# ttaoREtw/semi-tts

Measured on AMD Instinct MI355X. Metric: mel-frames/sec (decode+attn), higher is better.
Workload: dtype f32

## Files before the change

semi_tts_amd/csrc/attention.hip:

```cpp
#include "attention_body.h"

namespace {

inline unsigned at_align_bits(const AtArgs& a, const void* ws) {
    return (st_aligned16(a.pm) ? ST_ATTN_AL_PM : 0) | (st_aligned16(a.pq) ? ST_ATTN_AL_PQ : 0) | (st_aligned16(a.v) ? ST_ATTN_AL_V : 0) |
           (st_aligned16(a.loc_lin_w) ? ST_ATTN_AL_WL : 0) | (st_aligned16(a.memory) ? ST_ATTN_AL_MEM : 0) |
           (st_aligned16(a.s_buf) ? ST_ATTN_AL_S : 0) | (st_aligned16(ws) ? ST_ATTN_AL_WS : 0);
}

template <int PART>
int at_launch(const AtArgs& a, hipStream_t stream) {
    const AtPlan pl = at_plan(PART, a.B, a.L, a.A, a.E, a.F, a.K, PART == 1 ? a.pre_parts : PART == 2 ? a.fin_parts : 1, at_align_bits(a, nullptr));
    ST_CHECK_ARG(pl.code != ST_ATTN_R_DIMS, "attention step: bad dims");
    ST_CHECK_ARG(pl.code != ST_ATTN_R_K_EVEN, "attention step: location kernel size %d must be odd", a.K);
    ST_CHECK_ARG(pl.code != ST_ATTN_R_PARTS, "attention step: parts=%d must be 1, 2, 4 or 8 with E=%d a multiple of 4*parts", a.fin_parts, a.E);
    ST_CHECK_ARG(pl.code != ST_ATTN_R_E, "attention step: E=%d must be a multiple of 4 and <= %d", a.E, 4 * AT_THREADS);
    ST_CHECK_ARG(pl.code != ST_ATTN_R_ALIGN, "attention step: memory, pm/pq/v and the S buffer must be 16-byte aligned");
    ST_CHECK_ARG(PART == 1 || a.ctx || a.ctx_dst[0].base, "attention step: no context output");
    ST_CHECK_ARG(PART == 0 || a.s_buf, "attention step: S buffer missing");
    ST_CHECK_ARG(!a.h_q || (a.ada_std && a.ada_mean && a.h_adapt), "attention step: AdaIN pointers");
    const size_t lds_bytes = pl.lds;
    ST_CHECK_ARG(pl.code != ST_ATTN_R_LDS, "attention step: L=%d needs %zu B of LDS (> 160 KiB)%s", a.L, lds_bytes,
                 PART == 0 ? "; the split form (st_attn_pre_fwd with more parts + st_attn_fin_fwd) takes longer texts" : "");
    ST_CHECK_ARG(pl.code == 0, "attention step: refused (%d)", pl.code);
    static size_t configured[2] = {0, 0};
    int rc = st_lds_opt_in(reinterpret_cast<const void*>(at_kernel<true, PART>), 160 * 1024, pl.opt_in, configured[0]);
    if (!rc) rc = st_lds_opt_in(reinterpret_cast<const void*>(at_kernel<false, PART>), 160 * 1024, pl.opt_in, configured[1]);
    if (rc) return rc;
    const bool vec = pl.vec;
    const int nwg = pl.nwg;
    if (vec) hipLaunchKernelGGL((at_kernel<true, PART>), dim3(nwg), dim3(AT_THREADS), lds_bytes, stream, a.pq, a.pm, a.v, a.w_cum_prev, a.memory,
                                a.s_buf, a.L, a.A, a.E, a.fin_parts, a);
    else hipLaunchKernelGGL((at_kernel<false, PART>), dim3(nwg), dim3(AT_THREADS), lds_bytes, stream, a.pq, a.pm, a.v, a.w_cum_prev, a.memory,
                            a.s_buf, a.L, a.A, a.E, a.fin_parts, a);
    ST_LAUNCH_CHECK();
    return 0;
}

struct AsArgs {
    const float* pq; const float* s_buf; const float* memory; const float* v;
    float* w_tmp; int ld_w;
    float* ws;
    int B, L, A, E, P, Lp;
};

__global__ __launch_bounds__(AT_THREADS) void at_split_kernel(const AsArgs a) {
    __shared__ float es[512];
    __shared__ __attribute__((aligned(16))) float part[4 * AT_THREADS];
    __shared__ float stat[2];
    const int tid = threadIdx.x, lane = tid & 63, wave = tid >> 6;
    const int b = blockIdx.x / a.P, p = blockIdx.x - b * a.P;
    const int L = a.L, A = a.A, E = a.E;
    const int l0 = p * a.Lp, l1 = min(L, l0 + a.Lp), n = l1 - l0;
    const float* sb = a.s_buf + ((size_t)b * L + l0) * A;
    const float* memb = a.memory + ((size_t)b * L + l0) * E;
    const int ne4 = E >> 2;
    const int ng = AT_THREADS / ne4, e4 = tid % ne4, g = tid / ne4;
    constexpr int PFR = 11;
    f32x4 mpf[PFR];
#pragma unroll
    for (int j = 0; j < PFR; ++j) {
        const int l = g + j * ng;
        mpf[j] = (g < ng && l < n) ? st_ld4(memb + (size_t)l * E + e4 * 4) : f32x4{0.f, 0.f, 0.f, 0.f};
    }
// ... 218 lines not shown
```

semi_tts_amd/csrc/attention_body.h:

```cpp
#pragma once
#include "st_common.h"

#ifndef AT_PROF
#define AT_PROF(n)
#endif

namespace {

constexpr int AT_THREADS = 512;
constexpr int AT_WAVES = AT_THREADS / 64;
constexpr int AT_PF = 12;
constexpr int AT_LB = 8;
constexpr int AT_LP = 6;
constexpr int AT_CB = 4;
constexpr int AT_WLPF = 4;

struct AtArgs {
    const float* pq; const float* pm; const float* memory;
    const float* w_prev; int ld_wprev; const float* w_cum_prev;
    float* w_out; int ld_wout; float* w_cum_out;
    const float* loc_conv_w; const float* loc_lin_w; const float* v;
    float* ctx; int ld_ctx; st_t16_view ctx_dst[3];
    const float* h_q; int ld_hq; const float* ada_std; const float* ada_mean; float* h_adapt; int Q;
    float* s_buf;
// ... 6 lines not shown
};

constexpr int AT_GRAN_SPINS = 1 << 18;
__device__ __forceinline__ f32x4 at_wait_granules(const unsigned long long* base, unsigned epoch, int lane, int A, unsigned* status,
                                                  int max_spins) {
    typedef __attribute__((address_space(1))) unsigned long long gu64;
    gu64* gp = (gu64*)(base + min(lane * 4, A - 4));
    unsigned long long g0 = 0, g1 = 0, g2 = 0, g3 = 0;
    bool ok = false;
    for (int spins = 0; spins < max_spins; ++spins) {
        g0 = __hip_atomic_load(gp + 0, __ATOMIC_RELAXED, __HIP_MEMORY_SCOPE_AGENT);
        g1 = __hip_atomic_load(gp + 1, __ATOMIC_RELAXED, __HIP_MEMORY_SCOPE_AGENT);
        g2 = __hip_atomic_load(gp + 2, __ATOMIC_RELAXED, __HIP_MEMORY_SCOPE_AGENT);
        g3 = __hip_atomic_load(gp + 3, __ATOMIC_RELAXED, __HIP_MEMORY_SCOPE_AGENT);
        const bool mine = (unsigned)(g0 >> 32) == epoch && (unsigned)(g1 >> 32) == epoch &&
                          (unsigned)(g2 >> 32) == epoch && (unsigned)(g3 >> 32) == epoch;
        ok = __all(mine);
        if (ok) break;
        __builtin_amdgcn_s_sleep(2);
    }
    if (!ok && lane == 0 && status) __hip_atomic_fetch_or(status, 1u, __ATOMIC_RELAXED, __HIP_MEMORY_SCOPE_AGENT);
    const float nanv = __builtin_nanf("");
    return ok ? f32x4{__uint_as_float((unsigned)g0), __uint_as_float((unsigned)g1), __uint_as_float((unsigned)g2),
                      __uint_as_float((unsigned)g3)}
              : f32x4{nanv, nanv, nanv, nanv};
}

struct AtLds {
    int wt, wt_ld, wc, kp, hs, hl, cf, cf_ld, e, part, total;
};

__host__ __device__ inline int at_pos_per(int L, int nparts) {
    return nparts > 1 ? (((L + nparts - 1) / nparts + 11) / 12) * 12 : L;
}

__host__ __device__ inline AtLds at_layout(int L, int A, int E, int F, int K, int part = 0, int Lr = 0, bool pre_mfma = false) {
    AtLds o;
    int p = 0;
    const int Lh = part == 1 ? Lr : L;
    o.wt_ld = ((A + 3) & ~3) + 4;
    o.wt = p; if (part == 0 || (part == 1 && !pre_mfma)) p += F * o.wt_ld;
    o.kp = K <= 32 ? 32 : ((K + 3) & ~3);
    o.wc = p; if (part != 2) p += F * 2 * o.kp;
    o.hl = ((Lh + AT_CB + o.kp + 3) + 3) & ~3;
    o.hs = p; if (part != 2) p += 2 * o.hl;
    o.cf_ld = ((((Lh + AT_LP - 1) / AT_LP) * AT_LP + AT_CB + 3) & ~3) + (part == 1 ? 16 : 0);
    o.cf = p; if (part != 2) p += F * o.cf_ld;
    o.e = p; p += ((L + 3) & ~3);
    o.part = p; p += 4 * AT_THREADS;
    o.total = p;
    return o;
}

__device__ __forceinline__ float at_tanh(float x) {
    const float t = __expf(-2.0f * fabsf(x));
    return copysignf(__fdividef(1.0f - t, 1.0f + t), x);
}

__device__ __forceinline__ size_t at_t16_off(int b, int k, int KB) {
    return (((size_t)(b >> 4) * KB + (k >> 4)) * 64 + ((k >> 2) & 3) * 16 + (b & 15)) * 4 + (k & 3);
}

__device__ __forceinline__ void at_put_granule(unsigned long long* p, float v, unsigned epoch) {
    typedef __attribute__((address_space(1))) unsigned long long gu64;
    __hip_atomic_store((gu64*)p, ((unsigned long long)epoch << 32) | (unsigned long long)__float_as_uint(v), __ATOMIC_RELAXED,
                       __HIP_MEMORY_SCOPE_AGENT);
// ... 111 lines not shown
        float s = 0.0f;
        for (int gg = 0; gg < ng; ++gg) s += part[gg * E + e];
        at_put_granule(xme + e, s, a.epoch);
    }
    const int Es = E / P;
    if (wave < P) {
        const unsigned long long* xq = a.xchg + ((size_t)b * P + wave) * (E + 4);
        const f32x4 st4 = at_wait_granules(xq + E, a.epoch, lane, 4, a.status, AT_GRAN_SPINS);
        const f32x4 c4 = at_wait_granules(xq + (size_t)p * Es, a.epoch, lane, Es, a.status, AT_GRAN_SPINS);
        if (lane * 4 < Es) *reinterpret_cast<f32x4*>(cb + wave * 256 + lane * 4) = c4;
        if (lane == 0) { gst[2 * wave] = st4[0]; gst[2 * wave + 1] = st4[1]; }
    }
    __syncthreads();
    float M = -INFINITY;
    for (int q = 0; q < P; ++q) M = fmaxf(M, gst[2 * q]);
    float D = 0.0f;
    for (int q = 0; q < P; ++q) D += gst[2 * q + 1] * __expf(gst[2 * q] - M);
    if (tid < Es) {
        float s = 0.0f;
        for (int q = 0; q < P; ++q) s = fmaf(__expf(gst[2 * q] - M) / D, cb[q * 256 + tid], s);
        const int e = p * Es + tid;
#pragma unroll
        for (int d = 0; d < 3; ++d)
            if (a.ctx_dst[d].base) a.ctx_dst[d].base[at_t16_off(b, a.ctx_dst[d].kb0 * 16 + e, a.ctx_dst[d].kb_stride)] = s;
    }
    const float scp = __expf(stat[0] - M) / D;
    for (int l = tid; l < n; l += NT) {
        const float w = es[l] * scp;
        a.w_out[(size_t)b * a.ld_wout + l0 + l] = w;
        a.w_cum_out[(size_t)b * L + l0 + l] = w + a.w_cum_prev[(size_t)b * L + l0 + l];
    }
}

template <bool VEC, int PART, int NT = AT_THREADS, bool GRAN = false>
__device__ __forceinline__ void at_body(const AtArgs& a, const int wg, float* lds) {
    static_assert(!GRAN || (PART == 2 && VEC), "granule hand-off: fin part, vector form only");
    constexpr int NWV = NT / 64;
    constexpr int PFR = AT_PF * (AT_THREADS / NT);
    constexpr int NPB = PART == 2 ? AT_THREADS / NT : 0;
    const int nparts = (PART == 1 && a.pre_parts > 1) ? a.pre_parts : (PART == 2 && a.fin_parts > 1) ? a.fin_parts : 1;
    const int pshift = 31 - __builtin_clz((unsigned)nparts);
    const int b = wg >> pshift, ipart = wg & (nparts - 1);
#define AT_TOUCH(x) asm volatile("" :: "s"(x))
    AT_TOUCH(a.pq); AT_TOUCH(a.pm); AT_TOUCH(a.memory); AT_TOUCH(a.w_prev); AT_TOUCH(a.ld_wprev); AT_TOUCH(a.w_cum_prev);
    AT_TOUCH(a.s_buf); AT_TOUCH(a.w_out); AT_TOUCH(a.w_cum_out); AT_TOUCH(a.ld_wout);
    AT_TOUCH(a.loc_conv_w); AT_TOUCH(a.loc_lin_w); AT_TOUCH(a.v); AT_TOUCH(a.L); AT_TOUCH(a.A); AT_TOUCH(a.E); AT_TOUCH(a.F); AT_TOUCH(a.K);
#undef AT_TOUCH
    const int tid = threadIdx.x, lane = tid & 63, wave = tid >> 6;
    const int L = a.L, A = a.A, E = a.E, F = a.F, K = a.K;
    const int pos_per = PART == 1 ? at_pos_per(L, nparts) : L;
    const int pos_lo = PART == 1 ? min(L, ipart * pos_per) : 0, pos_hi = min(L, pos_lo + pos_per);
    const AtLds o = at_layout(L, A, E, F, K, PART, pos_per, PART == 1 && VEC && F == 32 && (A & 15) == 0);
    const int lb = PART == 1 ? pos_lo : 0;
    float* Wt = lds + o.wt;
    float* Wc = lds + o.wc;
    float* hs = lds + o.hs;
    float* cf = lds + o.cf;
    float* es = lds + o.e;
    float* part = lds + o.part;
    const int pad = (K - 1) / 2;

    AT_PROF(0);
    const float* pmb = (PART == 2 ? a.s_buf : a.pm) + (size_t)b * L * A;
    const float* pqb = a.pq + (size_t)b * A;
    f32x4 pf_pm4[NPB > 0 ? NPB : 1][AT_LP], pf_pq4 = {0.f, 0.f, 0.f, 0.f}, pf_v4 = {0.f, 0.f, 0.f, 0.f};
    float pf_cum = 0.0f;
    const bool pf_ok = PART == 2 && VEC && lane * 4 < A;
    if (PART == 2 && VEC) {
#pragma unroll
        for (int i = 0; i < NPB; ++i) {
#pragma unroll
            for (int j = 0; j < AT_LP; ++j) {
                const int l = min((wave + i * NWV) * AT_LP + j, L - 1);
                pf_pm4[i][j] = st_ld4(pmb + (size_t)l * A + min(lane * 4, A - 4));
            }
        }
        if (!GRAN) pf_pq4 = st_ld4(pqb + min(lane * 4, A - 4));
        pf_v4 = st_ld4(a.v + min(lane * 4, A - 4));
        if (wave == 0) pf_cum = a.w_cum_prev[(size_t)b * L + min(lane, L - 1)];
    }
    const int Es = PART == 2 ? E >> pshift : E;
    const int e_lo = PART == 2 ? ipart * Es : 0;
    const int ne4 = Es >> 2;
    int ng, e4, g;
    if ((ne4 & (ne4 - 1)) == 0) {
        const int sh = 31 - __builtin_clz((unsigned)ne4);
        ng = NT >> sh; e4 = tid & (ne4 - 1); g = tid >> sh;
    } else {
        ng = NT / ne4; e4 = tid % ne4; g = tid / ne4;
    }
    const bool ctx_active = g < ng;
    const float* memb = a.memory + (size_t)b * L * E;
    f32x4 mpf[PFR];
    if (PART != 1) {
        const __amdgpu_buffer_rsrc_t mrs = __builtin_amdgcn_make_buffer_rsrc((void*)memb, 0, L * E * 4, 0x00020000);
        const int v0 = ctx_active ? (g * E + e_lo + e4 * 4) * 4 : 0x7ffffff0;
        const int vstep = ng * E * 4;
#pragma unroll
        for (int j = 0; j < PFR; ++j)
            mpf[j] = __builtin_bit_cast(f32x4, __builtin_amdgcn_raw_buffer_load_b128(mrs, ctx_active ? v0 + j * vstep : v0, 0, 0));
    }

    if (GRAN) {
        if (wave == 0) {
            const f32x4 q4 = at_wait_granules(a.pq_gran + (size_t)b * A, a.epoch, lane, A, a.status, AT_GRAN_SPINS);
            if (lane * 4 < A) *reinterpret_cast<f32x4*>(part + lane * 4) = q4;
        }
        __syncthreads();
        pf_pq4 = *reinterpret_cast<const f32x4*>(part + min(lane * 4, A - 4));
    }
    AT_PROF(1);
    const bool wl_vec = VEC || ((F & 3) == 0 && st_aligned16(a.loc_lin_w));
    const int f4n = F >> 2;
    const int KP = o.kp;
    f32x4 wl4[AT_WLPF];
    constexpr int SM_MT = 2, SM_NT = 3;
    const bool s_mfma = PART == 1 && VEC && F == 32 && (A & 15) == 0;
    const int sm_g = lane >> 4, sm_n = lane & 15;
    const int sm_ntile = (pos_hi - pos_lo + 15) >> 4;
    float sm_aw[SM_MT][8];
    f32x4 sm_pm[SM_MT][SM_NT];
    const float* sm_pmb = a.pm + (size_t)b * L * A;
    if (PART != 2) {
    if (wl_vec && !s_mfma) {
#pragma unroll
        for (int j = 0; j < AT_WLPF; ++j) {
            const int idx = tid + j * NT;
            wl4[j] = idx < A * f4n ? st_ld4(a.loc_lin_w + (size_t)idx * 4) : f32x4{0.f, 0.f, 0.f, 0.f};
        }
    }
    {
        const int nwc = F * 2 * KP, nhs = 2 * o.hl;
        float wcv[4], hv[2];
#pragma unroll
        for (int j = 0; j < 4; ++j) {
            const int idx = tid + j * NT;
            const int row = idx / KP, k = idx - row * KP;
            wcv[j] = (idx < nwc && k < K) ? a.loc_conv_w[row * K + k] : 0.0f;
        }
#pragma unroll
        for (int j = 0; j < 2; ++j) {
            const int idx = tid + j * NT;
            const int c = idx / o.hl, p = idx - c * o.hl, l = lb + p - pad;
            float v = 0.0f;
            if (idx < nhs && l >= 0 && l < L) v = c == 0 ? a.w_prev[(size_t)b * a.ld_wprev + l] : a.w_cum_prev[(size_t)b * L + l];
            hv[j] = v;
        }
#pragma unroll
        for (int j = 0; j < 4; ++j) { const int idx = tid + j * NT; if (idx < nwc) Wc[idx] = wcv[j]; }
#pragma unroll
        for (int j = 0; j < 2; ++j) { const int idx = tid + j * NT; if (idx < nhs) hs[idx] = hv[j]; }
        for (int idx = tid + 4 * NT; idx < nwc; idx += NT) {
            const int row = idx / KP, k = idx - row * KP;
            Wc[idx] = k < K ? a.loc_conv_w[row * K + k] : 0.0f;
        }
        for (int idx = tid + 2 * NT; idx < nhs; idx += NT) {
            const int c = idx / o.hl, p = idx - c * o.hl, l = lb + p - pad;
            float v = 0.0f;
            if (l >= 0 && l < L) v = c == 0 ? a.w_prev[(size_t)b * a.ld_wprev + l] : a.w_cum_prev[(size_t)b * L + l];
            hs[idx] = v;
        }
    }
    }
    if (a.h_q && ipart == 0) {
        for (int j = tid; j < a.Q; j += NT) {
            const size_t q = (size_t)b * a.Q + j;
            a.h_adapt[q] = a.ada_std[q] * (a.h_q[(size_t)b * a.ld_hq + j] - a.ada_mean[q]);
        }
    }
    AT_PROF(2);
    if (PART != 2) st_lds_barrier();
    AT_PROF(3);

    if (PART == 1 && VEC) {
        const int wmax = A * F - 8, pmax = L * A - 4;
#pragma unroll
        for (int i = 0; i < SM_MT; ++i) {
            const int a0 = max(min(wave + i * NWV, (A >> 4) - 1), 0) * 16;
            const int wi = max(min((a0 + sm_n) * F + sm_g * 8, wmax), 0) & ~3;
            const f32x4 w0 = st_ld4(a.loc_lin_w + wi);
            const f32x4 w1 = st_ld4(a.loc_lin_w + wi + 4);
            sm_aw[i][0] = w0[0]; sm_aw[i][1] = w0[1]; sm_aw[i][2] = w0[2]; sm_aw[i][3] = w0[3];
            sm_aw[i][4] = w1[0]; sm_aw[i][5] = w1[1]; sm_aw[i][6] = w1[2]; sm_aw[i][7] = w1[3];
#pragma unroll
            for (int j = 0; j < SM_NT; ++j) {
                const int l = min(pos_lo + j * 16 + sm_n, L - 1);
                sm_pm[i][j] = st_ld4(sm_pmb + (min(l * A + a0 + 4 * sm_g, pmax) & ~3));
            }
        }
    }
    if (PART != 2) {
    {
        const int nlb = (pos_hi - pos_lo + AT_CB - 1) / AT_CB;
        for (int idx = tid; idx < F * nlb; idx += NT) {
            const int f = idx / nlb, l0 = pos_lo + (idx - f * nlb) * AT_CB;
            float acc0 = 0.f, acc1 = 0.f, acc2 = 0.f, acc3 = 0.f;
            if (KP == 32) {
#pragma unroll
                for (int c = 0; c < 2; ++c) {
                    const f32x4* hq = reinterpret_cast<const f32x4*>(hs + c * o.hl + (l0 - lb));
                    const f32x4* wq = reinterpret_cast<const f32x4*>(Wc + (f * 2 + c) * 32);
#pragma unroll
                    for (int kc = 0; kc < 4; ++kc) {
                        float h[12], w[8];
#pragma unroll
                        for (int j = 0; j < 3; ++j) { const f32x4 t = hq[2 * kc + j]; h[4 * j] = t[0]; h[4 * j + 1] = t[1]; h[4 * j + 2] = t[2]; h[4 * j + 3] = t[3]; }
#pragma unroll
                        for (int j = 0; j < 2; ++j) { const f32x4 t = wq[2 * kc + j]; w[4 * j] = t[0]; w[4 * j + 1] = t[1]; w[4 * j + 2] = t[2]; w[4 * j + 3] = t[3]; }
#pragma unroll
                        for (int k = 0; k < 8; ++k) {
                            acc0 = fmaf(w[k], h[k], acc0); acc1 = fmaf(w[k], h[k + 1], acc1);
                            acc2 = fmaf(w[k], h[k + 2], acc2); acc3 = fmaf(w[k], h[k + 3], acc3);
                        }
                    }
                }
            } else {
                for (int c = 0; c < 2; ++c) {
                    const float* h = hs + c * o.hl + (l0 - lb);
                    const float* w = Wc + (f * 2 + c) * KP;
                    float h0 = h[0], h1 = h[1], h2 = h[2];
#pragma unroll 8
                    for (int k = 0; k < K; ++k) {
                        const float h3 = h[k + 3];
// ... 34 lines not shown
            const f32x4 w4 = st_ld4(a.loc_lin_w + (size_t)idx * 4);
            Wt[(f0 + 0) * o.wt_ld + aa] = w4[0]; Wt[(f0 + 1) * o.wt_ld + aa] = w4[1];
            Wt[(f0 + 2) * o.wt_ld + aa] = w4[2]; Wt[(f0 + 3) * o.wt_ld + aa] = w4[3];
        }
    } else {
        for (int idx = tid; idx < A * F; idx += NT) {
            const int aa = idx / F, f = idx - aa * F;
            Wt[f * o.wt_ld + aa] = a.loc_lin_w[idx];
        }
    }
    }
    AT_PROF(4);
    if (PART != 2) st_lds_barrier();
    AT_PROF(5);

    if (PART == 1 && s_mfma) {
        auto sm_tile = [&](const int a0, const int nt, const float (&aw)[8], const f32x4 pm4) __attribute__((always_inline)) {
            const int l0 = pos_lo + nt * 16, l = l0 + sm_n;
            const float* cfp = cf + (sm_g * 8) * o.cf_ld + (l0 - lb) + sm_n;
            f32x4 acc = {0.f, 0.f, 0.f, 0.f};
#pragma unroll
            for (int k = 0; k < 8; ++k) acc = __builtin_amdgcn_mfma_f32_16x16x4f32(aw[k], cfp[k * o.cf_ld], acc, 0, 0, 0);
            if (l < pos_hi) {
                const f32x4 sv = {acc[0] + pm4[0], acc[1] + pm4[1], acc[2] + pm4[2], acc[3] + pm4[3]};
                *reinterpret_cast<f32x4*>(a.s_buf + ((size_t)b * L + l) * A + a0 + 4 * sm_g) = sv;
            }
        };
#pragma unroll
        for (int i = 0; i < SM_MT; ++i) {
            const int mt = wave + i * NWV;
            if (mt >= (A >> 4)) break;
#pragma unroll
            for (int j = 0; j < SM_NT; ++j)
                if (j < sm_ntile) sm_tile(mt * 16, j, sm_aw[i], sm_pm[i][j]);
            for (int j = SM_NT; j < sm_ntile; ++j) {
                const int l = min(pos_lo + j * 16 + sm_n, L - 1);
                sm_tile(mt * 16, j, sm_aw[i], st_ld4(sm_pmb + (size_t)l * A + mt * 16 + 4 * sm_g));
            }
        }
        for (int mt = wave + SM_MT * NWV; mt < (A >> 4); mt += NWV) {
            const int a0 = mt * 16;
            const f32x4 w0 = st_ld4(a.loc_lin_w + (size_t)(a0 + sm_n) * 32 + sm_g * 8);
            const f32x4 w1 = st_ld4(a.loc_lin_w + (size_t)(a0 + sm_n) * 32 + sm_g * 8 + 4);
            const float aw[8] = {w0[0], w0[1], w0[2], w0[3], w1[0], w1[1], w1[2], w1[3]};
            for (int j = 0; j < sm_ntile; ++j) {
                const int l = min(pos_lo + j * 16 + sm_n, L - 1);
                sm_tile(a0, j, aw, st_ld4(sm_pmb + (size_t)l * A + a0 + 4 * sm_g));
            }
        }
        return;
    }

    auto energy_block = [&](const int l0, const f32x4* pf) __attribute__((always_inline)) {
        float esum[AT_LB];
#pragma unroll
        for (int j = 0; j < AT_LB; ++j) esum[j] = 0.0f;
        for (int a0 = lane * 4; a0 < A; a0 += 256) {
            const int rem = A - a0;
            f32x4 pm4[AT_LP], pq4, v4;
            if (pf && pf_ok && a0 == lane * 4) {
#pragma unroll
                for (int j = 0; j < AT_LP; ++j) pm4[j] = pf[j];
                pq4 = pf_pq4;
                v4 = pf_v4;
            } else if (VEC) {
#pragma unroll
                for (int j = 0; j < AT_LP; ++j) {
                    const int l = l0 + j < L ? l0 + j : L - 1;
                    pm4[j] = st_ld4(pmb + (size_t)l * A + a0);
                }
                pq4 = GRAN ? pf_pq4 : st_ld4(pqb + a0);
                v4 = st_ld4(a.v + a0);
            } else {
#pragma unroll
                for (int j = 0; j < AT_LP; ++j) {
                    const int l = l0 + j < L ? l0 + j : L - 1;
                    pm4[j] = st_ld4_guard(pmb + (size_t)l * A + a0, rem);
                }
                pq4 = st_ld4_guard(pqb + a0, rem);
                v4 = st_ld4_guard(a.v + a0, rem);
            }
            f32x4 loc[AT_LP];
// ... 102 lines not shown
    if (ctx_active) {
        f32x4 acc = {0.f, 0.f, 0.f, 0.f};
#pragma unroll
        for (int j = 0; j < PFR; ++j) {
            const int l = g + j * ng;
            const float wv = es[min(l, L - 1)];
            const float w = l < L ? wv : 0.0f;
            acc[0] = fmaf(w, mpf[j][0], acc[0]); acc[1] = fmaf(w, mpf[j][1], acc[1]);
            acc[2] = fmaf(w, mpf[j][2], acc[2]); acc[3] = fmaf(w, mpf[j][3], acc[3]);
        }
        for (int l = g + PFR * ng; l < L; l += ng) {
            const f32x4 m4 = st_ld4(memb + (size_t)l * E + e_lo + e4 * 4);
            const float w = es[l];
            acc[0] = fmaf(w, m4[0], acc[0]); acc[1] = fmaf(w, m4[1], acc[1]);
            acc[2] = fmaf(w, m4[2], acc[2]); acc[3] = fmaf(w, m4[3], acc[3]);
        }
        *reinterpret_cast<f32x4*>(part + (size_t)(g * ne4 + e4) * 4) = acc;
    }
    AT_PROF(10);
    st_lds_barrier();
    AT_PROF(11);
    for (int e = tid; e < Es; e += NT) {
        float s = 0.0f;
        for (int gg = 0; gg < ng; ++gg) s += part[gg * Es + e];
        if (a.ctx) a.ctx[(size_t)b * a.ld_ctx + e_lo + e] = s;
#pragma unroll
        for (int d = 0; d < 3; ++d)
            if (a.ctx_dst[d].base) a.ctx_dst[d].base[at_t16_off(b, a.ctx_dst[d].kb0 * 16 + e_lo + e, a.ctx_dst[d].kb_stride)] = s;
    }
    AT_PROF(12);
}


template <bool VEC, int PART, int NT = AT_THREADS>
__global__ __launch_bounds__(NT) void at_kernel(const float* pq, const float* pm, const float* v, const float* w_cum_prev, const float* memory,
                                                float* s_buf, const int L, const int A, const int E, const int fin_parts, const AtArgs rest) {
    extern __shared__ __attribute__((aligned(16))) float at_lds[];
    AtArgs a = rest;
    a.pq = pq; a.pm = pm; a.v = v; a.w_cum_prev = w_cum_prev; a.memory = memory; a.s_buf = s_buf; a.L = L; a.A = A; a.E = E; a.fin_parts = fin_parts;
    at_body<VEC, PART, NT>(a, blockIdx.x, at_lds);
}

inline int at_pre_parts_eff(int parts) { return (parts >= 2 && parts <= 64 && (parts & (parts - 1)) == 0) ? parts : 1; }
inline bool at_fin_parts_ok(int parts, int E) { return parts == 1 || ((parts == 2 || parts == 4 || parts == 8) && E % (4 * parts) == 0); }

inline int at_ctx_dst_fill(AtArgs& a, const st_t16_view* ctx_dst, int n_ctx_dst, const char* who) {
    ST_CHECK_ARG(n_ctx_dst >= 0 && n_ctx_dst <= 3, "%s: n_ctx_dst=%d", who, n_ctx_dst);
    for (int d = 0; d < n_ctx_dst; ++d) a.ctx_dst[d] = ctx_dst[d];
    return 0;
}

inline int at_step_fill(AtArgs& a, const st_attn_step_job* j, int B, const char* who) {
    ST_CHECK_ARG(j, "%s: null job", who);
    ST_CHECK_ARG(!j->h_q || j->n_ctx_dst == 0, "%s: AdaIN and T16 context destinations do not go together", who);
    memset(&a, 0, sizeof(a));
    if (at_ctx_dst_fill(a, j->ctx_dst, j->n_ctx_dst, who)) return -1;
    a.pq = j->pq; a.pm = j->pm; a.memory = j->memory; a.w_prev = j->w_prev; a.ld_wprev = j->ld_wprev; a.w_cum_prev = j->w_cum_prev;
    a.w_out = j->w_out; a.ld_wout = j->ld_wout; a.w_cum_out = j->w_cum_out;
    a.loc_conv_w = j->loc_conv_w; a.loc_lin_w = j->loc_lin_w; a.v = j->v; a.ctx = j->ctx; a.ld_ctx = j->ld_ctx;
    a.h_q = j->h_q; a.ld_hq = j->ld_hq; a.ada_std = j->ada_std; a.ada_mean = j->ada_mean; a.h_adapt = j->h_adapt; a.Q = j->Q;
    a.B = B; a.L = j->L; a.A = j->A; a.E = j->E; a.F = j->F; a.K = j->K;
    return 0;
}

inline int at_pre_fill(AtArgs& a, const st_attn_pre_job* j, int B, const char* who) {
    ST_CHECK_ARG(j && j->pm && j->w_prev && j->w_cum_prev && j->loc_conv_w && j->loc_lin_w && j->L > 0 && j->A > 0 && j->F > 0 && j->K > 0 &&
                 (j->K & 1), "%s: bad attention job", who);
    memset(&a, 0, sizeof(a));
    a.pm = j->pm; a.w_prev = j->w_prev; a.ld_wprev = j->ld_wprev; a.w_cum_prev = j->w_cum_prev;
    a.loc_conv_w = j->loc_conv_w; a.loc_lin_w = j->loc_lin_w; a.s_buf = j->s_buf; a.cf_out = j->cf_out;
    a.pre_parts = at_pre_parts_eff(j->parts);
    a.B = B; a.L = j->L; a.A = j->A; a.E = 4; a.F = j->F; a.K = j->K;
    return 0;
// ... 83 lines not shown
```

semi_tts_amd/csrc/skinny_packed.hip:

```cpp
#include "st_common.h"
#include "attention_body.h"
#include "attention_bwd_body.h"
#include <cstdlib>

#ifndef PK_PROF
#define PK_PROF(n)
#endif
#ifndef RT2_PROF
#define RT2_PROF(n)
#endif

namespace {

constexpr int PK_MAXSEG = 3;

__host__ __device__ inline int pk_kb(int k) { return (k + 15) >> 4; }

struct PackArgs {
    const float* w[PK_MAXSEG]; int ldw[PK_MAXSEG]; int k[PK_MAXSEG]; int kb0[PK_MAXSEG];
    int nseg; int N; int H; int KB; int tiles; float* out;
};

__device__ __forceinline__ void pack_weight_body(const PackArgs& a);
__global__ __launch_bounds__(256) void pack_weight_kernel(const PackArgs a) { pack_weight_body(a); }
// ... 834 lines not shown
    const int half = __builtin_amdgcn_readfirstlane((int)threadIdx.x / (KW * 64));
    if (exp_ == 1 && i < n_ab) return;
    if (exp_ == 2 && i >= n_ab) return;
    if (i < n_ab) {
        if (half) return;
        const int part = i / ab.B;
        ab_body<true, LBLK, NS>(ab, i - part * ab.B, pk_dyn_lds, part);
        return;
    }
    PkArgs a = rest;
    a.w = w; a.x = x; a.w_kbs = w_kbs; a.x_kbs = x_kbs; a.KB = KB; a.B = B; a.N = N; a.H = 0;
    pk_body<2, 1, KW, TRIP>(a, i - n_ab, half, red + half * KW * 64, &pw, half * KW * 64);
}

template <int MODE, int NB, int KW, int TRIP>
__global__ __launch_bounds__(KW * 64) void pk_pw_hist_kernel(const f32x4* w, const f32x4* x, const int w_kbs, const int x_kbs, const int KB,
                                                             const int B, const int N, const int tiles_a, const int n_h, const int n_sum,
                                                             const PkArgs rest, const PkPw pw, const AbHistArgs hist, const PkSumArgs sum, const int exp_) {
    extern __shared__ __attribute__((aligned(16))) float pk_dyn_lds[];
    __shared__ f32x4 red[KW * NB * 64];
    const int i = blockIdx.x;
    if (exp_ == 3 && i < n_h) return;
    if (exp_ == 4 && i >= n_h && i < n_h + n_sum) return;
    if (exp_ == 5 && i >= n_h + n_sum) return;
    if (i < n_h) { ab_hist_body(hist, i, pk_dyn_lds); return; }
    if (i < n_h + n_sum) { pk_sum_body(sum, i - n_h, KW * 64); return; }
    PkArgs a = rest;
    a.w = w; a.x = x; a.w_kbs = w_kbs; a.x_kbs = x_kbs; a.KB = KB; a.B = B; a.N = N; a.H = 0;
    const int j = i - n_h - n_sum;
    const int by = j / tiles_a;
    pk_body<MODE, NB, KW, TRIP>(a, j - by * tiles_a, by, red, MODE == 2 ? &pw : nullptr);
}

template <int NB, int KW, int TRIP, bool VEC>
__global__ __launch_bounds__(KW * 64) void pk_attnpre_kernel(const f32x4* w, const f32x4* x, const int w_kbs, const int x_kbs, const int KB,
                                                             const int B, const int N, const int tiles_a, const int n_lin,
                                                             const float* at_pm, const float* at_wprev, const int at_L,
                                                             const PkArgs a_rest, const AtArgs t_rest) {
    extern __shared__ __attribute__((aligned(16))) float pk_dyn_lds[];
    __shared__ f32x4 red[KW * NB * 64];
    PkArgs a = a_rest;
    a.w = w; a.x = x; a.w_kbs = w_kbs; a.x_kbs = x_kbs; a.KB = KB; a.B = B; a.N = N;
    AtArgs t = t_rest;
    t.pm = at_pm; t.w_prev = at_wprev; t.L = at_L;
    static_assert(KW * 64 == AT_THREADS, "both parts use 512-thread workgroups");
    const int i = blockIdx.x;
    if (i < n_lin) {
        const int by = n_lin <= 2 * tiles_a ? (i >= tiles_a ? 1 : 0) : i / tiles_a;
        pk_body<1, NB, KW, TRIP>(a, i - by * tiles_a, by, red);
    }
    else at_body<VEC, 1>(t, i - n_lin, pk_dyn_lds);
}

template <int NB, int KW, int TRIP, bool VEC>
__global__ __launch_bounds__(KW * 64) void pk_attnpre_part_kernel(const f32x4* w, const f32x4* x, const int w_kbs, const int x_kbs, const int KB,
                                                                  const int B, const int N, const int tiles_a, const int n_lin,
                                                                  const float* at_pm, const float* at_wprev, const int at_L,
                                                                  const PkArgs a_rest, const AtArgs t_rest, const int n_at, const PkPartArgs p) {
    extern __shared__ __attribute__((aligned(16))) float pk_dyn_lds[];
    __shared__ f32x4 red[KW * NB * 64];
    static_assert(KW * 64 == AT_THREADS, "both parts use 512-thread workgroups");
    const int i = blockIdx.x;
    if (i < n_lin) {
        PkArgs a = a_rest;
        a.w = w; a.x = x; a.w_kbs = w_kbs; a.x_kbs = x_kbs; a.KB = KB; a.B = B; a.N = N;
        const int by = n_lin <= 2 * tiles_a ? (i >= tiles_a ? 1 : 0) : i / tiles_a;
        pk_body<1, NB, KW, TRIP>(a, i - by * tiles_a, by, red);
    } else if (i < n_lin + n_at) {
        AtArgs t = t_rest;
        t.pm = at_pm; t.w_prev = at_wprev; t.L = at_L;
        at_body<VEC, 1>(t, i - n_lin, pk_dyn_lds);
    } else pk_part_body<KW, 2>(p, i - n_lin - n_at, reinterpret_cast<f32x4*>(pk_dyn_lds));
}


template <int NB, int KW, int TRIP>
__global__ __launch_bounds__(KW * 64) void pk_attnfin_kernel(const f32x4* w, const f32x4* x, const int w_kbs, const int x_kbs, const int KB,
                                                             const int B, const int N, const int tiles_a, const int n_lin,
                                                             const PkArgs a_rest, const AtArgs t) {
    extern __shared__ __attribute__((aligned(16))) float pk_dyn_lds[];
    __shared__ f32x4 red[KW * NB * 64];
    static_assert(KW * 64 == AT_THREADS, "both parts use 512-thread workgroups");
    const int i = blockIdx.x;
    if (i < n_lin) {
        PkArgs a = a_rest;
        a.w = w; a.x = x; a.w_kbs = w_kbs; a.x_kbs = x_kbs; a.KB = KB; a.B = B; a.N = N;
        const int by = n_lin <= 2 * tiles_a ? (i >= tiles_a ? 1 : 0) : i / tiles_a;
        pk_body<1, NB, KW, TRIP>(a, i - by * tiles_a, by, red);
    }
    else at_body<true, 2, AT_THREADS, true>(t, i - n_lin, pk_dyn_lds);
}

template <int NB, int KW, int TRIP>
__global__ __launch_bounds__(KW * 64) void pk_attnfin_part_kernel(const f32x4* w, const f32x4* x, const int w_kbs, const int x_kbs, const int KB,
                                                                  const int B, const int N, const int tiles_a, const int n_lin,
                                                                  const PkArgs a_rest, const AtArgs t, const int n_att, const PkPartArgs p) {
    extern __shared__ __attribute__((aligned(16))) float pk_dyn_lds[];
    __shared__ f32x4 red[KW * NB * 64];
    static_assert(KW * 64 == AT_THREADS, "both parts use 512-thread workgroups");
    const int i = blockIdx.x;
    if (i < n_lin) {
        PkArgs a = a_rest;
        a.w = w; a.x = x; a.w_kbs = w_kbs; a.x_kbs = x_kbs; a.KB = KB; a.B = B; a.N = N;
        const int by = n_lin <= 2 * tiles_a ? (i >= tiles_a ? 1 : 0) : i / tiles_a;
// ... 35 lines not shown
    const int BT = (B + 15) >> 4;
    if (mode == 0 && pk_rt2_shape(B, tiles)) return PkPlan{ST_PK_LSTM_RT2, BT == 2 ? 1 : 2, tiles / 2, 2, 0};
    int nb;
    if (mode == 1) {
        nb = 1;
        while (nb < 4 && nb < BT && tiles * ((BT + nb - 1) / nb) > 512) ++nb;
    } else nb = BT < 4 ? BT : 4;
    return PkPlan{ST_PK_KERNEL, nb, tiles, (BT + nb - 1) / nb, 0};
}

inline bool pk_pair_shape(int B0, int H0, int B1, int H1) {
    return pk_rt2_shape(B0, H0 / 4) && pk_rt2_shape(B1, H1 / 4) && ((B0 + 15) >> 4) == 2 && ((B1 + 15) >> 4) == 2 && H0 % 8 == 0 && H1 % 8 == 0;
}

inline bool pk_attnpre_vec(int A, int F, bool aligned) { return (A % 4 == 0) && (F % 4 == 0) && aligned; }

inline PkPlan pk_attnpre_plan(int B, int tiles, int n_at, int part_n, bool vec) {
    const int BT = (B + 15) >> 4;
    const int nb = (part_n > 0 || BT == 1 || tiles <= 128) ? 1 : (BT < 4 ? BT : 4);
    const int gy = (BT + nb - 1) / nb;
    return PkPlan{part_n > 0 ? ST_PK_ATTNPRE_PART : ST_PK_ATTNPRE, nb, tiles * gy + n_at + (part_n >> 5), 1, vec ? 1 : 0};
}

template <int NB>
int pk_launch_attnpre(const PkArgs& a, int tiles, const AtArgs& t, const PkPlan& pl, hipStream_t st, const PkPartArgs* pp = nullptr) {
    constexpr int KW = 8, TRIP = NB == 1 ? PK_TRIP_SMALL : 2;
    const int BT = (a.B + 15) >> 4, gy = (BT + NB - 1) / NB;
    const bool vec = pl.vec != 0;
    const AtLds o = at_layout(t.L, t.A, t.E, t.F, t.K, 1, at_pos_per(t.L, t.pre_parts > 1 ? t.pre_parts : 1), vec && t.F == 32 && t.A % 16 == 0);
    size_t lds = (size_t)o.total * sizeof(float);
    if (pp && lds < sizeof(f32x4) * KW * 4 * 64) lds = sizeof(f32x4) * KW * 4 * 64;
    ST_CHECK_ARG(lds + sizeof(f32x4) * KW * NB * 64 <= 160 * 1024, "linear + attention-pre launch: L=%d needs too much LDS (use more parts)", t.L);
    const int n_at = t.B * (t.pre_parts > 1 ? t.pre_parts : 1);
    if constexpr (NB == 1) if (pp) {
        auto kern = vec ? pk_attnpre_part_kernel<NB, KW, TRIP, true> : pk_attnpre_part_kernel<NB, KW, TRIP, false>;
        static size_t configured[2] = {0, 0};
        if (int rc = st_lds_opt_in(reinterpret_cast<const void*>(kern), lds, lds > 32 * 1024, configured[vec ? 1 : 0])) return rc;
        hipLaunchKernelGGL(kern, dim3(pl.gx), dim3(KW * 64), lds, st, a.w, a.x, a.w_kbs, a.x_kbs,
                           a.KB, a.B, a.N, tiles, tiles * gy, t.pm, t.w_prev, t.L, a, t, n_at, *pp);
        ST_LAUNCH_CHECK();
        return 0;
    }
    auto kern = vec ? pk_attnpre_kernel<NB, KW, TRIP, true> : pk_attnpre_kernel<NB, KW, TRIP, false>;
    static size_t configured[2] = {0, 0};
    if (int rc = st_lds_opt_in(reinterpret_cast<const void*>(kern), lds, lds > 48 * 1024, configured[vec ? 1 : 0])) return rc;
    hipLaunchKernelGGL(kern, dim3(pl.gx), dim3(KW * 64), lds, st, a.w, a.x, a.w_kbs, a.x_kbs,
                       a.KB, a.B, a.N, tiles, tiles * gy, t.pm, t.w_prev, t.L, a, t);
    ST_LAUNCH_CHECK();
    return 0;
}

template <int MODE, int NB>
int pk_launch(const PkArgs& a, const PkPlan& pl, hipStream_t st) {
    constexpr int KW = 8, TRIP = (MODE == 1 && NB == 1) ? PK_TRIP_SMALL : 2;
    dim3 grid(pl.gx, pl.gy);
    hipLaunchKernelGGL((pk_kernel<MODE, NB, KW, TRIP>), grid, dim3(KW * 64), 0, st, a.w, a.x, a.w_kbs, a.x_kbs, a.KB, a.B, a.N, a.H, a);
    ST_LAUNCH_CHECK();
    return 0;
}

#ifndef PK_LSTM_KW
#define PK_LSTM_KW 8
#endif
#ifndef PK_LSTM_TRIP
#define PK_LSTM_TRIP 2
#endif
template <int MODE>
int pk_dispatch(const PkArgs& a, int tiles, hipStream_t st) {
    const PkPlan pl = pk_plan(MODE, a.B, tiles);
    if (pl.family == ST_PK_LSTM_RT2) {
        if constexpr (MODE == 0) {
        constexpr int LKW = PK_LSTM_KW, LTR = PK_LSTM_TRIP;
        const dim3 grid(pl.gx, pl.gy);
#if defined(PK_AUX_Q0) || defined(PK_AUX_D0)
        if (pl.nb == 1 && a.KB > 128)
            hipLaunchKernelGGL((pk_lstm_rt2_kernel<LKW, LTR, 1, PK_AUX_D0, PK_AUX_D1>), grid, dim3(LKW * 64), 0, st, a.w, a.x, a.w_kbs, a.x_kbs, a.KB, a.B, a.H, a);
        else if (pl.nb == 1)
            hipLaunchKernelGGL((pk_lstm_rt2_kernel<LKW, LTR, 1, PK_AUX_Q0, PK_AUX_Q1>), grid, dim3(LKW * 64), 0, st, a.w, a.x, a.w_kbs, a.x_kbs, a.KB, a.B, a.H, a);
// ... 665 lines not shown
```

Baseline: 2.895 million.

## Issue score-tile prefetch before LDS staging and specialize prefetch depth by part length

Moves the loads of the pm tiles and attention weights for the MFMA score step so they are issued before the conv-weight and history LDS stores rather than after the barrier. The global-load latency then overlaps the staging work. Adds a template parameter for how many position tiles are prefetched (1-3), picked on the host from the per-part position count, so short parts use fewer registers and do not load unused tiles. It also replaces a division with a shift or compare in index math. The extra s_barrier inside the prefetch and the larger number of kernel instantiations add some risk.

```diff
diff --git a/semi_tts_amd/csrc/attention.hip b/semi_tts_amd/csrc/attention.hip
--- a/semi_tts_amd/csrc/attention.hip
+++ b/semi_tts_amd/csrc/attention.hip
@@ -23,13 +23,20 @@
     ST_CHECK_ARG(pl.code != ST_ATTN_R_LDS, "attention step: L=%d needs %zu B of LDS (> 160 KiB)%s", a.L, lds_bytes,
                  PART == 0 ? "; the split form (st_attn_pre_fwd with more parts + st_attn_fin_fwd) takes longer texts" : "");
     ST_CHECK_ARG(pl.code == 0, "attention step: refused (%d)", pl.code);
-    static size_t configured[2] = {0, 0};
-    int rc = st_lds_opt_in(reinterpret_cast<const void*>(at_kernel<true, PART>), 160 * 1024, pl.opt_in, configured[0]);
-    if (!rc) rc = st_lds_opt_in(reinterpret_cast<const void*>(at_kernel<false, PART>), 160 * 1024, pl.opt_in, configured[1]);
+    using AtKernel = decltype(&at_kernel<true, PART>);
+    AtKernel kerns[4] = {at_kernel<true, PART>, nullptr, nullptr, nullptr};
+    if constexpr (PART == 1) {
+        kerns[1] = at_kernel<true, 1, AT_THREADS, 1>; kerns[2] = at_kernel<true, 1, AT_THREADS, 2>; kerns[3] = kerns[0];
+    }
+    const int kv = PART == 1 ? at_pre_tiles(a.L, pl.parts) : 0;
+    static size_t configured[5] = {0, 0, 0, 0, 0};
+    int rc = st_lds_opt_in(reinterpret_cast<const void*>(at_kernel<false, PART>), 160 * 1024, pl.opt_in, configured[4]);
+    for (int i = 0; i < (PART == 1 ? 3 : 1) && !rc; ++i)
+        rc = st_lds_opt_in(reinterpret_cast<const void*>(kerns[i]), 160 * 1024, pl.opt_in, configured[i]);
     if (rc) return rc;
     const bool vec = pl.vec;
     const int nwg = pl.nwg;
-    if (vec) hipLaunchKernelGGL((at_kernel<true, PART>), dim3(nwg), dim3(AT_THREADS), lds_bytes, stream, a.pq, a.pm, a.v, a.w_cum_prev, a.memory,
+    if (vec) hipLaunchKernelGGL(kerns[kv], dim3(nwg), dim3(AT_THREADS), lds_bytes, stream, a.pq, a.pm, a.v, a.w_cum_prev, a.memory,
                                 a.s_buf, a.L, a.A, a.E, a.fin_parts, a);
     else hipLaunchKernelGGL((at_kernel<false, PART>), dim3(nwg), dim3(AT_THREADS), lds_bytes, stream, a.pq, a.pm, a.v, a.w_cum_prev, a.memory,
                             a.s_buf, a.L, a.A, a.E, a.fin_parts, a);
diff --git a/semi_tts_amd/csrc/attention_body.h b/semi_tts_amd/csrc/attention_body.h
--- a/semi_tts_amd/csrc/attention_body.h
+++ b/semi_tts_amd/csrc/attention_body.h
@@ -62,6 +62,11 @@
 
 __host__ __device__ inline int at_pos_per(int L, int nparts) {
     return nparts > 1 ? (((L + nparts - 1) / nparts + 11) / 12) * 12 : L;
+}
+
+__host__ __device__ inline int at_pre_tiles(int L, int nparts) {
+    const int n = at_pos_per(L, nparts);
+    return n <= 16 ? 1 : n <= 32 ? 2 : 3;
 }
 
 __host__ __device__ inline AtLds at_layout(int L, int A, int E, int F, int K, int part = 0, int Lr = 0, bool pre_mfma = false) {
@@ -239,9 +244,10 @@
     }
 }
 
-template <bool VEC, int PART, int NT = AT_THREADS, bool GRAN = false>
+template <bool VEC, int PART, int NT = AT_THREADS, bool GRAN = false, int SNT = 3>
 __device__ __forceinline__ void at_body(const AtArgs& a, const int wg, float* lds) {
     static_assert(!GRAN || (PART == 2 && VEC), "granule hand-off: fin part, vector form only");
+    static_assert(SNT >= 1 && SNT <= 3 && (SNT == 3 || (PART == 1 && VEC)), "prefetched position tiles: 1..3, chosen for the vector pre part only");
     constexpr int NWV = NT / 64;
     constexpr int PFR = AT_PF * (AT_THREADS / NT);
     constexpr int NPB = PART == 2 ? AT_THREADS / NT : 0;
@@ -255,7 +261,7 @@
 #undef AT_TOUCH
     const int tid = threadIdx.x, lane = tid & 63, wave = tid >> 6;
     const int L = a.L, A = a.A, E = a.E, F = a.F, K = a.K;
-    const int pos_per = PART == 1 ? at_pos_per(L, nparts) : L;
+    const int pos_per = (PART == 1 && nparts > 1) ? ((((L + nparts - 1) >> pshift) + 11) / 12) * 12 : L;
     const int pos_lo = PART == 1 ? min(L, ipart * pos_per) : 0, pos_hi = min(L, pos_lo + pos_per);
     const AtLds o = at_layout(L, A, E, F, K, PART, pos_per, PART == 1 && VEC && F == 32 && (A & 15) == 0);
     const int lb = PART == 1 ? pos_lo : 0;
@@ -321,65 +327,15 @@
     const int f4n = F >> 2;
     const int KP = o.kp;
     f32x4 wl4[AT_WLPF];
-    constexpr int SM_MT = 2, SM_NT = 3;
+    constexpr int SM_MT = 2, SM_NT = SNT;
     const bool s_mfma = PART == 1 && VEC && F == 32 && (A & 15) == 0;
     const int sm_g = lane >> 4, sm_n = lane & 15;
     const int sm_ntile = (pos_hi - pos_lo + 15) >> 4;
     float sm_aw[SM_MT][8];
     f32x4 sm_pm[SM_MT][SM_NT];
     const float* sm_pmb = a.pm + (size_t)b * L * A;
-    if (PART != 2) {
-    if (wl_vec && !s_mfma) {
-#pragma unroll
-        for (int j = 0; j < AT_WLPF; ++j) {
-            const int idx = tid + j * NT;
-            wl4[j] = idx < A * f4n ? st_ld4(a.loc_lin_w + (size_t)idx * 4) : f32x4{0.f, 0.f, 0.f, 0.f};
-        }
-    }
-    {
-        const int nwc = F * 2 * KP, nhs = 2 * o.hl;
-        float wcv[4], hv[2];
-#pragma unroll
-        for (int j = 0; j < 4; ++j) {
-            const int idx = tid + j * NT;
-            const int row = idx / KP, k = idx - row * KP;
-            wcv[j] = (idx < nwc && k < K) ? a.loc_conv_w[row * K + k] : 0.0f;
-        }
-#pragma unroll
-        for (int j = 0; j < 2; ++j) {
-            const int idx = tid + j * NT;
-            const int c = idx / o.hl, p = idx - c * o.hl, l = lb + p - pad;
-            float v = 0.0f;
-            if (idx < nhs && l >= 0 && l < L) v = c == 0 ? a.w_prev[(size_t)b * a.ld_wprev + l] : a.w_cum_prev[(size_t)b * L + l];
-            hv[j] = v;
-        }
-#pragma unroll
-        for (int j = 0; j < 4; ++j) { const int idx = tid + j * NT; if (idx < nwc) Wc[idx] = wcv[j]; }
-#pragma unroll
-        for (int j = 0; j < 2; ++j) { const int idx = tid + j * NT; if (idx < nhs) hs[idx] = hv[j]; }
-        for (int idx = tid + 4 * NT; idx < nwc; idx += NT) {
-            const int row = idx / KP, k = idx - row * KP;
-            Wc[idx] = k < K ? a.loc_conv_w[row * K + k] : 0.0f;
-        }
-        for (int idx = tid + 2 * NT; idx < nhs; idx += NT) {
-            const int c = idx / o.hl, p = idx - c * o.hl, l = lb + p - pad;
-            float v = 0.0f;
-            if (l >= 0 && l < L) v = c == 0 ? a.w_prev[(size_t)b * a.ld_wprev + l] : a.w_cum_prev[(size_t)b * L + l];
-            hs[idx] = v;
-        }
-    }
-    }
-    if (a.h_q && ipart == 0) {
-        for (int j = tid; j < a.Q; j += NT) {
-            const size_t q = (size_t)b * a.Q + j;
-            a.h_adapt[q] = a.ada_std[q] * (a.h_q[(size_t)b * a.ld_hq + j] - a.ada_mean[q]);
-        }
-    }
-    AT_PROF(2);
-    if (PART != 2) st_lds_barrier();
-    AT_PROF(3);
-
-    if (PART == 1 && VEC) {
+    auto sm_request = [&]() __attribute__((always_inline)) {
+        asm volatile("s_barrier" ::: "memory");
         const int wmax = A * F - 8, pmax = L * A - 4;
 #pragma unroll
         for (int i = 0; i < SM_MT; ++i) {
@@ -395,7 +351,67 @@
                 sm_pm[i][j] = st_ld4(sm_pmb + (min(l * A + a0 + 4 * sm_g, pmax) & ~3));
             }
         }
-    }
+    };
+    if (PART != 2) {
+    if (wl_vec && !s_mfma) {
+#pragma unroll
+        for (int j = 0; j < AT_WLPF; ++j) {
+            const int idx = tid + j * NT;
+            wl4[j] = idx < A * f4n ? st_ld4(a.loc_lin_w + (size_t)idx * 4) : f32x4{0.f, 0.f, 0.f, 0.f};
+        }
+    }
+    {
+        const int nwc = F * 2 * KP, nhs = 2 * o.hl;
+        float wcv[4], hv[2];
+        int wrow[4];
+        if (KP == 32) {
+#pragma unroll
+            for (int j = 0; j < 4; ++j) wrow[j] = (tid + j * NT) >> 5;
+        } else {
+#pragma unroll
+            for (int j = 0; j < 4; ++j) wrow[j] = (tid + j * NT) / KP;
+        }
+#pragma unroll
+        for (int j = 0; j < 4; ++j) {
+            const int idx = tid + j * NT;
+            const int row = wrow[j], k = idx - row * KP;
+            wcv[j] = (idx < nwc && k < K) ? a.loc_conv_w[row * K + k] : 0.0f;
+        }
+#pragma unroll
+        for (int j = 0; j < 2; ++j) {
+            const int idx = tid + j * NT;
+            const int c = idx >= o.hl ? 1 : 0, p = idx - c * o.hl, l = lb + p - pad;
+            float v = 0.0f;
+            if (idx < nhs && l >= 0 && l < L) v = c == 0 ? a.w_prev[(size_t)b * a.ld_wprev + l] : a.w_cum_prev[(size_t)b * L + l];
+            hv[j] = v;
+        }
+        AT_PROF(2);
+        if (PART == 1 && VEC) sm_request();
+#pragma unroll
+        for (int j = 0; j < 4; ++j) { const int idx = tid + j * NT; if (idx < nwc) Wc[idx] = wcv[j]; }
+#pragma unroll
+        for (int j = 0; j < 2; ++j) { const int idx = tid + j * NT; if (idx < nhs) hs[idx] = hv[j]; }
+        for (int idx = tid + 4 * NT; idx < nwc; idx += NT) {
+            const int row = idx / KP, k = idx - row * KP;
+            Wc[idx] = k < K ? a.loc_conv_w[row * K + k] : 0.0f;
+        }
+        for (int idx = tid + 2 * NT; idx < nhs; idx += NT) {
+            const int c = idx / o.hl, p = idx - c * o.hl, l = lb + p - pad;
+            float v = 0.0f;
+            if (l >= 0 && l < L) v = c == 0 ? a.w_prev[(size_t)b * a.ld_wprev + l] : a.w_cum_prev[(size_t)b * L + l];
+            hs[idx] = v;
+        }
+    }
+    }
+    if (a.h_q && ipart == 0) {
+        for (int j = tid; j < a.Q; j += NT) {
+            const size_t q = (size_t)b * a.Q + j;
+            a.h_adapt[q] = a.ada_std[q] * (a.h_q[(size_t)b * a.ld_hq + j] - a.ada_mean[q]);
+        }
+    }
+    if (PART == 2) { AT_PROF(2); }
+    if (PART != 2) st_lds_barrier();
+    AT_PROF(3);
     if (PART != 2) {
     {
         const int nlb = (pos_hi - pos_lo + AT_CB - 1) / AT_CB;
@@ -496,7 +512,10 @@
             if (mt >= (A >> 4)) break;
 #pragma unroll
             for (int j = 0; j < SM_NT; ++j)
-                if (j < sm_ntile) sm_tile(mt * 16, j, sm_aw[i], sm_pm[i][j]);
+                if (j < sm_ntile) {
+                    sm_tile(mt * 16, j, sm_aw[i], sm_pm[i][j]);
+                    if (i == 0 && j == 0) AT_PROF(6);
+                }
             for (int j = SM_NT; j < sm_ntile; ++j) {
                 const int l = min(pos_lo + j * 16 + sm_n, L - 1);
                 sm_tile(mt * 16, j, sm_aw[i], st_ld4(sm_pmb + (size_t)l * A + mt * 16 + 4 * sm_g));
@@ -512,6 +531,7 @@
                 sm_tile(a0, j, aw, st_ld4(sm_pmb + (size_t)l * A + a0 + 4 * sm_g));
             }
         }
+        AT_PROF(7);
         return;
     }
 
@@ -680,13 +700,13 @@
 }
 
 
-template <bool VEC, int PART, int NT = AT_THREADS>
+template <bool VEC, int PART, int NT = AT_THREADS, int SNT = 3>
 __global__ __launch_bounds__(NT) void at_kernel(const float* pq, const float* pm, const float* v, const float* w_cum_prev, const float* memory,
                                                 float* s_buf, const int L, const int A, const int E, const int fin_parts, const AtArgs rest) {
     extern __shared__ __attribute__((aligned(16))) float at_lds[];
     AtArgs a = rest;
     a.pq = pq; a.pm = pm; a.v = v; a.w_cum_prev = w_cum_prev; a.memory = memory; a.s_buf = s_buf; a.L = L; a.A = A; a.E = E; a.fin_parts = fin_parts;
-    at_body<VEC, PART, NT>(a, blockIdx.x, at_lds);
+    at_body<VEC, PART, NT, false, SNT>(a, blockIdx.x, at_lds);
 }
 
 inline int at_pre_parts_eff(int parts) { return (parts >= 2 && parts <= 64 && (parts & (parts - 1)) == 0) ? parts : 1; }
diff --git a/semi_tts_amd/csrc/skinny_packed.hip b/semi_tts_amd/csrc/skinny_packed.hip
--- a/semi_tts_amd/csrc/skinny_packed.hip
+++ b/semi_tts_amd/csrc/skinny_packed.hip
@@ -890,7 +890,7 @@
     pk_body<MODE, NB, KW, TRIP>(a, j - by * tiles_a, by, red, MODE == 2 ? &pw : nullptr);
 }
 
-template <int NB, int KW, int TRIP, bool VEC>
+template <int NB, int KW, int TRIP, bool VEC, int SNT = 3>
 __global__ __launch_bounds__(KW * 64) void pk_attnpre_kernel(const f32x4* w, const f32x4* x, const int w_kbs, const int x_kbs, const int KB,
                                                              const int B, const int N, const int tiles_a, const int n_lin,
                                                              const float* at_pm, const float* at_wprev, const int at_L,
@@ -907,10 +907,10 @@
         const int by = n_lin <= 2 * tiles_a ? (i >= tiles_a ? 1 : 0) : i / tiles_a;
         pk_body<1, NB, KW, TRIP>(a, i - by * tiles_a, by, red);
     }
-    else at_body<VEC, 1>(t, i - n_lin, pk_dyn_lds);
-}
-
-template <int NB, int KW, int TRIP, bool VEC>
+    else at_body<VEC, 1, AT_THREADS, false, SNT>(t, i - n_lin, pk_dyn_lds);
+}
+
+template <int NB, int KW, int TRIP, bool VEC, int SNT = 3>
 __global__ __launch_bounds__(KW * 64) void pk_attnpre_part_kernel(const f32x4* w, const f32x4* x, const int w_kbs, const int x_kbs, const int KB,
                                                                   const int B, const int N, const int tiles_a, const int n_lin,
                                                                   const float* at_pm, const float* at_wprev, const int at_L,
@@ -927,7 +927,7 @@
     } else if (i < n_lin + n_at) {
         AtArgs t = t_rest;
         t.pm = at_pm; t.w_prev = at_wprev; t.L = at_L;
-        at_body<VEC, 1>(t, i - n_lin, pk_dyn_lds);
+        at_body<VEC, 1, AT_THREADS, false, SNT>(t, i - n_lin, pk_dyn_lds);
     } else pk_part_body<KW, 2>(p, i - n_lin - n_at, reinterpret_cast<f32x4*>(pk_dyn_lds));
 }
 
@@ -1029,18 +1029,25 @@
     if (pp && lds < sizeof(f32x4) * KW * 4 * 64) lds = sizeof(f32x4) * KW * 4 * 64;
     ST_CHECK_ARG(lds + sizeof(f32x4) * KW * NB * 64 <= 160 * 1024, "linear + attention-pre launch: L=%d needs too much LDS (use more parts)", t.L);
     const int n_at = t.B * (t.pre_parts > 1 ? t.pre_parts : 1);
+    const int kv = vec ? at_pre_tiles(t.L, t.pre_parts > 1 ? t.pre_parts : 1) : 0;
     if constexpr (NB == 1) if (pp) {
-        auto kern = vec ? pk_attnpre_part_kernel<NB, KW, TRIP, true> : pk_attnpre_part_kernel<NB, KW, TRIP, false>;
-        static size_t configured[2] = {0, 0};
-        if (int rc = st_lds_opt_in(reinterpret_cast<const void*>(kern), lds, lds > 32 * 1024, configured[vec ? 1 : 0])) return rc;
+        using Kern = decltype(&pk_attnpre_part_kernel<NB, KW, TRIP, false>);
+        const Kern kerns[4] = {pk_attnpre_part_kernel<NB, KW, TRIP, false>, pk_attnpre_part_kernel<NB, KW, TRIP, true, 1>,
+                               pk_attnpre_part_kernel<NB, KW, TRIP, true, 2>, pk_attnpre_part_kernel<NB, KW, TRIP, true, 3>};
+        const Kern kern = kerns[kv];
+        static size_t configured[4] = {0, 0, 0, 0};
+        if (int rc = st_lds_opt_in(reinterpret_cast<const void*>(kern), lds, lds > 32 * 1024, configured[kv])) return rc;
         hipLaunchKernelGGL(kern, dim3(pl.gx), dim3(KW * 64), lds, st, a.w, a.x, a.w_kbs, a.x_kbs,
                            a.KB, a.B, a.N, tiles, tiles * gy, t.pm, t.w_prev, t.L, a, t, n_at, *pp);
         ST_LAUNCH_CHECK();
         return 0;
     }
-    auto kern = vec ? pk_attnpre_kernel<NB, KW, TRIP, true> : pk_attnpre_kernel<NB, KW, TRIP, false>;
-    static size_t configured[2] = {0, 0};
-    if (int rc = st_lds_opt_in(reinterpret_cast<const void*>(kern), lds, lds > 48 * 1024, configured[vec ? 1 : 0])) return rc;
+    using Kern = decltype(&pk_attnpre_kernel<NB, KW, TRIP, false>);
+    const Kern kerns[4] = {pk_attnpre_kernel<NB, KW, TRIP, false>, pk_attnpre_kernel<NB, KW, TRIP, true, 1>,
+                           pk_attnpre_kernel<NB, KW, TRIP, true, 2>, pk_attnpre_kernel<NB, KW, TRIP, true, 3>};
+    const Kern kern = kerns[kv];
+    static size_t configured[4] = {0, 0, 0, 0};
+    if (int rc = st_lds_opt_in(reinterpret_cast<const void*>(kern), lds, lds > 48 * 1024, configured[kv])) return rc;
     hipLaunchKernelGGL(kern, dim3(pl.gx), dim3(KW * 64), lds, st, a.w, a.x, a.w_kbs, a.x_kbs,
                        a.KB, a.B, a.N, tiles, tiles * gy, t.pm, t.w_prev, t.L, a, t);
     ST_LAUNCH_CHECK();
```

After: 2.905 million (median of 6 runs). No clear change (+0.3%).
